# codenotary/immustore

Hardware: AMD Instinct MI355X
Metric: device-resident GiB/s hashed, htree build, 1M x 1KiB leaves (higher is better)
Workload: dtype u32; 1 GPU

## Files before the change

### immustore_amd/csrc/htree_kernels.hip

```cpp
#include <algorithm>
#include <cstring>

#include "mh_internal.hpp"
#include "sha256_cdna.hpp"
#include "digest_io.hpp"

typedef __attribute__((address_space(3))) void lds_void_t;
typedef __attribute__((address_space(1))) void glb_void_t;

namespace mh {

void LevelGeom::init(uint64_t n_) {
    n = n_;
    nlevels = 0;
    total = 0;
    for (int l = 0; l < kMaxLevels; l++) off[l] = width[l] = 0;
    if (n == 0) return;
    uint64_t w = n;
    for (;;) {
        off[nlevels] = total;
        width[nlevels] = w;
        total += w;
        nlevels++;
        if (w == 1) break;
        w = (w + 1) / 2;
    }
}

static LevelArgs level_args(const LevelGeom &g) {
    LevelArgs a;
    for (int l = 0; l < kMaxLevels; l++) {
        a.off[l] = g.off[l];
        a.width[l] = l < g.nlevels ? g.width[l] : 0;
    }
    return a;
}

void pad_block_kw(uint64_t len, KWTable *out) {
    static const uint32_t K[64] = {
        0x428a2f98u, 0x71374491u, 0xb5c0fbcfu, 0xe9b5dba5u, 0x3956c25bu, 0x59f111f1u, 0x923f82a4u,
        0xab1c5ed5u, 0xd807aa98u, 0x12835b01u, 0x243185beu, 0x550c7dc3u, 0x72be5d74u, 0x80deb1feu,
        0x9bdc06a7u, 0xc19bf174u, 0xe49b69c1u, 0xefbe4786u, 0x0fc19dc6u, 0x240ca1ccu, 0x2de92c6fu,
        0x4a7484aau, 0x5cb0a9dcu, 0x76f988dau, 0x983e5152u, 0xa831c66du, 0xb00327c8u, 0xbf597fc7u,
        0xc6e00bf3u, 0xd5a79147u, 0x06ca6351u, 0x14292967u, 0x27b70a85u, 0x2e1b2138u, 0x4d2c6dfcu,
        0x53380d13u, 0x650a7354u, 0x766a0abbu, 0x81c2c92eu, 0x92722c85u, 0xa2bfe8a1u, 0xa81a664bu,
        0xc24b8b70u, 0xc76c51a3u, 0xd192e819u, 0xd6990624u, 0xf40e3585u, 0x106aa070u, 0x19a4c116u,
        0x1e376c08u, 0x2748774cu, 0x34b0bcb5u, 0x391c0cb3u, 0x4ed8aa4au, 0x5b9cca4fu, 0x682e6ff3u,
        0x748f82eeu, 0x78a5636fu, 0x84c87814u, 0x8cc70208u, 0x90befffau, 0xa4506cebu, 0xbef9a3f7u,
        0xc67178f2u};
    auto ror = [](uint32_t x, int n) { return (x >> n) | (x << (32 - n)); };
    uint32_t w[64] = {0};
    uint64_t bits = len * 8;
    w[0] = 0x80000000u;
    w[14] = (uint32_t)(bits >> 32);
    w[15] = (uint32_t)bits;
    for (int t = 16; t < 64; t++) {
        uint32_t s0 = ror(w[t - 15], 7) ^ ror(w[t - 15], 18) ^ (w[t - 15] >> 3);
        uint32_t s1 = ror(w[t - 2], 17) ^ ror(w[t - 2], 19) ^ (w[t - 2] >> 10);
        w[t] = w[t - 16] + s0 + w[t - 7] + s1;
    }
    for (int t = 0; t < 64; t++) out->kw[t] = K[t] + w[t];
}

constexpr int kLaneLevels = 11;
struct LaneLevels {
    uint64_t off[kLaneLevels];
    uint64_t width[kLaneLevels];
};

static LaneLevels lane_levels(const LevelGeom &g) {
    LaneLevels a;
    for (int l = 0; l < kLaneLevels; l++) {
        a.off[l] = l < g.nlevels ? g.off[l] : 0;
        a.width[l] = l < g.nlevels ? g.width[l] : 0;
    }
    return a;
}

__device__ __forceinline__ void store_node(uint8_t *levels, const LaneLevels &la, int l, uint64_t q,
                                           const uint32_t w[8]) {
    if (q < la.width[l]) store_digest(levels + (la.off[l] + q) * 32, w);
}

template <int VER, int KW4>
__device__ __forceinline__ void digest_words(const uint32_t key[5], const uint32_t hv[8],
                                             uint32_t w[16]) {
    constexpr int P = VER == 1 ? 1 : 0;
    constexpr int L = (VER == 1 ? 4 : 0) + 4 * KW4 + 32;
#pragma unroll
    for (int j = 0; j < 16; j++) w[j] = 0;
    if (VER == 1) w[0] = 4 * KW4;
// ... 65 lines not shown
};

template <int LPL>
struct Log2 {
    static constexpr int v = LPL == 1 ? 0 : LPL == 2 ? 1 : 2;
};

constexpr int kFixedThreads = 256;
constexpr int kWaveLds = 8192;
constexpr uint32_t kFixedMaxValLen = 1u << 24;
constexpr uint32_t kFixedFastMaxValLen = 1u << 23;

#ifndef MH_WG_PROBE
#define MH_WG_PROBE(point)
#endif

__device__ __forceinline__ void dma_issue(const uint8_t *__restrict__ vals, uint32_t stride,
                                          uint64_t wave_slot0, int lpl, int i, uint64_t n,
                                          uint32_t byte_off, bool two, char *lds, int lane) {
    uint32_t ln = (uint32_t)lane;
    asm volatile("" : "+v"(ln));
    const uint64_t e0 = wave_slot0 * lpl;
    const uint32_t lim = (uint32_t)min<uint64_t>(n - 1 - e0, 0xffffffffull);
    const uint8_t *g0 = vals + e0 * stride + byte_off;
    if (two) {
        const uint32_t k2 = (ln & 7) ^ (ln >> 4);
#pragma unroll
        for (int j = 0; j < 8; j++) {
            const uint32_t rel = min((uint32_t)((j * 8 + (ln >> 3)) * lpl + i), lim);
            const uint32_t off = rel * stride + ((j & 1) ? (k2 ^ 4) : k2) * 16;
            __builtin_amdgcn_global_load_lds((glb_void_t *)(g0 + off),
                                             (lds_void_t *)(lds + j * 1024), 16, 0, 0);
        }
    } else {
        const uint32_t k1 = (ln & 3) ^ ((ln >> 4) & 3);
#pragma unroll
        for (int j = 0; j < 4; j++) {
            const uint32_t rel = min((uint32_t)((j * 16 + (ln >> 2)) * lpl + i), lim);
            const uint32_t off = rel * stride + k1 * 16;
            __builtin_amdgcn_global_load_lds((glb_void_t *)(g0 + off),
                                             (lds_void_t *)(lds + j * 1024), 16, 0, 0);
        }
    }
}

__device__ __forceinline__ void lds_block(const char *lds, int lane, bool two, int h,
                                          uint32_t w[16]) {
#pragma unroll
    for (int c = 0; c < 4; c++) {
        int addr;
        if (two) {
            const int k = 4 * h + c;
            addr = lane * 128 + ((k ^ ((lane >> 1) & 7)) << 4);
        } else {
            addr = lane * 64 + ((c ^ ((lane >> 2) & 3)) << 4);
        }
        const uint4 v = *reinterpret_cast<const uint4 *>(lds + addr);
        w[4 * c + 0] = bswap(v.x);
        w[4 * c + 1] = bswap(v.y);
        w[4 * c + 2] = bswap(v.z);
        w[4 * c + 3] = bswap(v.w);
    }
}

__device__ __forceinline__ void fast_lane_offsets(uint32_t stride, uint32_t lim, int lpl, int i,
                                                  int lane, uint32_t voff[8]) {
    const uint32_t ln = (uint32_t)lane;
    const uint32_t k2 = (ln & 7) ^ (ln >> 4);
#pragma unroll
    for (int j = 0; j < 8; j++) {
        const uint32_t rel = min((uint32_t)((j * 8 + (ln >> 3)) * lpl + i), lim);
        voff[j] = rel * stride + ((j & 1) ? (k2 ^ 4) : k2) * 16;
    }
}

__device__ __forceinline__ void dma_issue_fast(__amdgpu_buffer_rsrc_t rsrc, char *lds,
                                               const uint32_t voff[8], uint32_t byte_off) {
#pragma unroll
    for (int j = 0; j < 8; j++)
        __builtin_amdgcn_raw_ptr_buffer_load_lds(rsrc, (lds_void_t *)(lds + j * 1024), 16,
                                                 (int)voff[j], (int)byte_off, 0, 0);
}

__device__ __forceinline__ void lds_read4(const char *lds, uint32_t a, uint4 r[4]) {
#pragma unroll
    for (int c = 0; c < 4; c++) r[c] = *reinterpret_cast<const uint4 *>(lds + (a ^ (c << 4)));
}

__device__ __forceinline__ void swap_words(const uint4 r[4], uint32_t w[16]) {
#pragma unroll
    for (int c = 0; c < 4; c++) {
        w[4 * c + 0] = bswap(r[c].x);
        w[4 * c + 1] = bswap(r[c].y);
        w[4 * c + 2] = bswap(r[c].z);
        w[4 * c + 3] = bswap(r[c].w);
    }
}

enum : int { OP_VALUE = 0, OP_TAIL, OP_DIGEST, OP_LEAF, OP_NODE1, OP_NODE2 };

template <int LPL, bool FAST>
__global__ __launch_bounds__(kFixedThreads) void k_entries_fixed(
    const uint8_t *__restrict__ vals, uint32_t val_len, const uint8_t *__restrict__ keys,
    uint32_t key_len, int version, uint64_t n, uint8_t *__restrict__ hvals_out,
    uint8_t *__restrict__ levels, LaneLevels la, int wg_levels, KWTable kwt) {
    extern __shared__ __attribute__((aligned(16))) char smem[];
    const int lane = threadIdx.x & 63;
    int wave = threadIdx.x >> 6;
    if (FAST) wave = __builtin_amdgcn_readfirstlane(wave);
    uint32_t *kw_lds = reinterpret_cast<uint32_t *>(smem + (kFixedThreads / 64) * kWaveLds);
    if (FAST) {
        if (threadIdx.x < 64) kw_lds[threadIdx.x] = kwt.kw[threadIdx.x];
    } else if (threadIdx.x == 0) {
        uint32_t w[16];
#pragma unroll
        for (int j = 0; j < 16; j++) w[j] = 0;
        w[0] = 0x80000000u;
        const uint64_t bits = (uint64_t)val_len * 8;
        w[14] = (uint32_t)(bits >> 32);
        w[15] = (uint32_t)bits;
#pragma unroll
        for (int t = 0; t < 64; t++) {
            if (t >= 16)
                w[t & 15] = ssig1(w[(t - 2) & 15]) + w[(t - 7) & 15] + ssig0(w[(t - 15) & 15]) +
                            w[t & 15];
            kw_lds[t] = kK256[t] + w[t & 15];
        }
    }
    __syncthreads();
    MH_WG_PROBE(0);
    char *lds = smem + wave * kWaveLds;
    const uint64_t wave_slot0 = ((uint64_t)blockIdx.x * (kFixedThreads / 64) + wave) * 64;
    const uint64_t first = (wave_slot0 + lane) * LPL;
    const int c = first < n ? (int)min<uint64_t>(LPL, n - first) : 0;
    const bool wave_busy = wave_slot0 * LPL < n;

    const uint32_t nfull = val_len >> 6;
    const uint32_t rem = val_len & 63;
    const uint32_t nsteps2 = nfull >> 1;
    const uint32_t units = nsteps2 + (nfull & 1);
    const int kw4 = key_len >> 2;
    State s;
    s.init();
    uint32_t A[8], B[8], ny7 = 0;
    const bool fast_busy = FAST && wave_busy;
    const uint64_t e0 = fast_busy ? wave_slot0 * LPL : 0;
    const uint64_t ents = fast_busy ? n - e0 : 0;
    const uint32_t lim = ents - 1 < 0xffffffffull ? (uint32_t)(ents - 1) : 0xffffffffu;
    const uint64_t left = ents * val_len < 0xffffffffull ? ents * val_len : 0xffffffffull;
    const uint64_t base = (uint64_t)vals + e0 * val_len;
    const uint64_t base_s =
        ((uint64_t)(uint32_t)__builtin_amdgcn_readfirstlane((int)(uint32_t)(base >> 32)) << 32) |
        (uint32_t)__builtin_amdgcn_readfirstlane((int)(uint32_t)base);
    const __amdgpu_buffer_rsrc_t rsrc = __builtin_amdgcn_make_buffer_rsrc(
        (void *)base_s, 0, __builtin_amdgcn_readfirstlane((int)(uint32_t)left), 0x00020000);
    uint32_t voff[8];
    const uint32_t lds_a0 =
        (uint32_t)wave * kWaveLds + (uint32_t)lane * 128 + ((((uint32_t)lane >> 1) & 7) << 4);
    if (wave_busy) {
    if (FAST) {
        fast_lane_offsets(val_len, lim, LPL, 0, lane, voff);
        dma_issue_fast(rsrc, lds, voff, 0);
    } else {
    if (units) dma_issue(vals, val_len, wave_slot0, LPL, 0, n, 0, nsteps2 > 0, lds, lane);
    }

    int i = 0;
    uint32_t b = 0;
    int node = 0;
    int op = nfull ? OP_VALUE : (rem ? OP_TAIL : OP_DIGEST);
    if (!nfull && !rem && i < c) compress_kw(s, kw_lds);
    for (;;) {
        const uint64_t idx = first + i;
        bool on = i < c;
        if (op == OP_VALUE && FAST) {
#pragma unroll 1
            for (uint32_t bb = 0; bb < nfull; bb++) {
                uint4 r[4];
                uint32_t w[16];
                uint32_t a = lds_a0;
                asm volatile("" : "+v"(a));
                lds_read4(smem, a ^ ((bb & 1) << 6), r);
                if (bb & 1) {
                    asm volatile("s_waitcnt lgkmcnt(0)" ::: "memory");
                    const uint32_t u1 = (bb >> 1) + 1;
                    if (u1 < units) dma_issue_fast(rsrc, lds, voff, u1 * 128);
                }
                swap_words(r, w);
                compress(s, w);
                if (bb == 0 && i == 0) MH_WG_PROBE(3);
            }
            if (i + 1 < LPL) {
                fast_lane_offsets(val_len, lim, LPL, i + 1, lane, voff);
                dma_issue_fast(rsrc, lds, voff, 0);
            }
            if (on) compress_kw(s, kw_lds);
            op = OP_DIGEST;
            continue;
        }
        if (op == OP_VALUE) {
#pragma unroll 1
            for (; b < nfull; b++) {
                const uint32_t u = b >> 1;
                const bool two = u < nsteps2;
                const int h = two ? (int)(b & 1) : 0;
                uint32_t w[16];
                lds_block(lds, lane, two, h, w);
                if (!two || h == 1) {
                    asm volatile("s_waitcnt lgkmcnt(0)" ::: "memory");
                    if (u + 1 < units)
                        dma_issue(vals, val_len, wave_slot0, LPL, i, n, (u + 1) * 128,
                                  (u + 1) < nsteps2, lds, lane);
                    else if (i + 1 < LPL)
                        dma_issue(vals, val_len, wave_slot0, LPL, i + 1, n, 0, nsteps2 > 0, lds,
                                  lane);
                }
                if (on) compress(s, w);
                if (b == 0 && i == 0) MH_WG_PROBE(3);
            }
            b = 0;
            if (rem) {
                op = OP_TAIL;
            } else {
                if (on) compress_kw(s, kw_lds);
                op = OP_DIGEST;
            }
            continue;
        }
        uint32_t w[16];
        if (op == OP_TAIL) {
            const uint32_t rw = rem >> 2;
            const uint32_t *tp =
                reinterpret_cast<const uint32_t *>(vals + idx * val_len + (uint64_t)nfull * 64);
#pragma unroll
            for (int j = 0; j < 12; j++) w[j] = (on && j < (int)rw) ? bswap(tp[j]) : 0u;
#pragma unroll
            for (int j = 12; j < 16; j++) w[j] = 0;
#pragma unroll
            for (int j = 0; j < 13; j++)
                if (j == (int)rw) w[j] = 0x80000000u;
            const uint64_t bits = (uint64_t)val_len * 8;
            w[14] = (uint32_t)(bits >> 32);
            w[15] = (uint32_t)bits;
        } else if (op == OP_DIGEST) {
            if (on && hvals_out) store_digest(hvals_out + idx * 32, s.h);
            uint32_t key[5] = {0, 0, 0, 0, 0};
            const uint32_t *kp = reinterpret_cast<const uint32_t *>(keys + idx * key_len);
#pragma unroll
            for (int j = 0; j < 5; j++)
                if (on && j < kw4) key[j] = bswap(kp[j]);
            digest_block(version, kw4, key, s.h, w);
            s.init();
        } else if (op == OP_LEAF) {
            w[0] = s.h[0] >> 8;
#pragma unroll
            for (int j = 1; j < 8; j++) w[j] = __builtin_amdgcn_alignbit(s.h[j - 1], s.h[j], 8);
            w[8] = (s.h[7] << 24) | 0x00800000u;
#pragma unroll
            for (int j = 9; j < 15; j++) w[j] = 0;
            w[15] = 33u * 8u;
            s.init();
        } else if (op == OP_NODE1) {
            uint32_t l[8], r[8];
            if (LPL >= 2 && node == 0) {
#pragma unroll
                for (int j = 0; j < 8; j++) {
                    l[j] = i == 1 ? A[j] : B[j];
                    r[j] = s.h[j];
                }
                on = i < c;
            } else {
                copy8(l, A);
                copy8(r, B);
                on = c >= 3;
            }
            w[0] = 0x01000000u | (l[0] >> 8);
#pragma unroll
            for (int j = 1; j < 8; j++) w[j] = __builtin_amdgcn_alignbit(l[j - 1], l[j], 8);
            w[8] = __builtin_amdgcn_alignbit(l[7], r[0], 8);
#pragma unroll
            for (int j = 1; j < 8; j++) w[8 + j] = __builtin_amdgcn_alignbit(r[j - 1], r[j], 8);
            ny7 = r[7];
            s.init();
        } else {
            w[0] = (ny7 << 24) | 0x00800000u;
#pragma unroll
            for (int j = 1; j < 15; j++) w[j] = 0;
            w[15] = 65u * 8u;
            on = (node == 0) ? (i < c) : (c >= 3);
        }

        if (on) compress(s, w);

        bool entry_done = false;
        if (op == OP_TAIL) {
            op = OP_DIGEST;
        } else if (op == OP_DIGEST) {
            op = OP_LEAF;
        } else if (op == OP_LEAF) {
            if (i < c) store_digest(levels + idx * 32, s.h);
            if (LPL == 1) break;
            entry_done = true;
            if ((i & 1) == 0) {
#pragma unroll
                for (int j = 0; j < 8; j++) {
                    if (i == 0) A[j] = s.h[j];
                    else B[j] = s.h[j];
                }
            } else {
                node = 0;
                op = OP_NODE1;
                continue;
            }
        } else if (op == OP_NODE1) {
            op = OP_NODE2;
            continue;
        } else {
            const bool lane_on = (node == 0) ? (i < c) : (c >= 3);
            if (node == 0) {
#pragma unroll
                for (int j = 0; j < 8; j++) {
                    if (lane_on) {
                        if (i == 1) A[j] = s.h[j];
                        else B[j] = s.h[j];
                    }
                }
                if (c > 0) store_node(levels, la, 1, (first >> 1) + (i >> 1), i == 1 ? A : B);
                if (LPL == 4 && i == 3) {
                    node = 1;
                    op = OP_NODE1;
                    continue;
                }
            } else {
#pragma unroll
                for (int j = 0; j < 8; j++)
                    if (lane_on) A[j] = s.h[j];
            }
            if (LPL == 4 && i == 3 && c > 0) store_node(levels, la, 2, first >> 2, A);
            if (LPL == 2 || i == LPL - 1) break;
            entry_done = true;
        }
        if (entry_done) {
            if (++i >= LPL) break;
            s.init();
            op = nfull ? OP_VALUE : (rem ? OP_TAIL : OP_DIGEST);
            if (!nfull && !rem && i < c) compress_kw(s, kw_lds);
        }
    }
    }

    constexpr int L0 = LPL == 4 ? 2 : (LPL == 2 ? 1 : 0);
    MH_WG_PROBE(1);
    if (wg_levels == 0) return;
    const int t = threadIdx.x;
    uint32_t(*buf)[kFixedThreads][9] = reinterpret_cast<uint32_t(*)[kFixedThreads][9]>(smem);
    __syncthreads();
#pragma unroll
    for (int j = 0; j < 8; j++) buf[0][t][j] = LPL == 1 ? s.h[j] : A[j];
    int cur = 0;
#pragma unroll 1
    for (int st = 1; st <= wg_levels; st++) {
        __syncthreads();
        const int active = kFixedThreads >> st;
        const int l = L0 + st;
        if (t < active) {
            const uint64_t q = (uint64_t)blockIdx.x * active + t;
            if (q < la.width[l]) {
                uint32_t lft[8], rgt[8], out[8];
#pragma unroll
                for (int j = 0; j < 8; j++) lft[j] = buf[cur][2 * t][j];
                if (2 * q + 1 < la.width[l - 1]) {
#pragma unroll
                    for (int j = 0; j < 8; j++) rgt[j] = buf[cur][2 * t + 1][j];
                    node_hash(lft, rgt, out);
                } else {
                    copy8(out, lft);
                }
                store_digest(levels + (la.off[l] + q) * 32, out);
#pragma unroll
                for (int j = 0; j < 8; j++) buf[cur ^ 1][t][j] = out[j];
            }
        }
        cur ^= 1;
    }
    MH_WG_PROBE(2);
}

template <int LPL>
__global__ __launch_bounds__(256) void k_leaves_from_digests(const uint8_t *__restrict__ digests,
                                                             uint64_t n, uint8_t *__restrict__ levels,
                                                             LaneLevels la) {
    const uint64_t lane_id = (uint64_t)blockIdx.x * blockDim.x + threadIdx.x;
    const uint64_t first = lane_id * LPL;
    if (first >= n) return;
    const int c = (int)min<uint64_t>(LPL, n - first);
    LaneReducer<LPL> red;
#pragma unroll 1
    for (int i = 0; i < LPL; i++) {
        if (i < c) {
            uint32_t d[8], leaf[8];
            load_digest(digests + (first + i) * 32, d);
            leaf_hash(d, leaf);
            store_digest(levels + (first + i) * 32, leaf);
            red.push(i, leaf);
        }
    }
    red.finish(c, first, levels, la);
}

__global__ void k_copy_nodes(const uint8_t *__restrict__ src, uint64_t n, uint8_t *__restrict__ dst) {
    const uint64_t i = (uint64_t)blockIdx.x * blockDim.x + threadIdx.x;
    if (i < n * 2) reinterpret_cast<uint4 *>(dst)[i] = reinterpret_cast<const uint4 *>(src)[i];
}

template <int T>
__global__ __launch_bounds__(T) void k_reduce(uint8_t *__restrict__ levels, LevelArgs la, int l0,
                                              int nsteps, int top, uint8_t *__restrict__ root) {
    __shared__ uint32_t buf[2][T][9];
    const int t = threadIdx.x;
    const uint64_t blk = blockIdx.x;
    {
        const uint64_t q = blk * T + t;
        if (q < la.width[l0 + 1]) {
            uint32_t lft[8], rgt[8], out[8];
            load_digest(levels + (la.off[l0] + 2 * q) * 32, lft);
            if (2 * q + 1 < la.width[l0]) {
                load_digest(levels + (la.off[l0] + 2 * q + 1) * 32, rgt);
                node_hash_g(lft, rgt, out);
            } else {
                copy8(out, lft);
// ... 284 lines not shown
```

### immustore_amd/csrc/sha256_cdna.hpp

```cpp
#pragma once
#include <hip/hip_runtime.h>
#include <stdint.h>

namespace mh {

__device__ __constant__ static const uint32_t kK256[64] = {
    0x428a2f98u, 0x71374491u, 0xb5c0fbcfu, 0xe9b5dba5u, 0x3956c25bu, 0x59f111f1u, 0x923f82a4u,
    0xab1c5ed5u, 0xd807aa98u, 0x12835b01u, 0x243185beu, 0x550c7dc3u, 0x72be5d74u, 0x80deb1feu,
    0x9bdc06a7u, 0xc19bf174u, 0xe49b69c1u, 0xefbe4786u, 0x0fc19dc6u, 0x240ca1ccu, 0x2de92c6fu,
    0x4a7484aau, 0x5cb0a9dcu, 0x76f988dau, 0x983e5152u, 0xa831c66du, 0xb00327c8u, 0xbf597fc7u,
    0xc6e00bf3u, 0xd5a79147u, 0x06ca6351u, 0x14292967u, 0x27b70a85u, 0x2e1b2138u, 0x4d2c6dfcu,
    0x53380d13u, 0x650a7354u, 0x766a0abbu, 0x81c2c92eu, 0x92722c85u, 0xa2bfe8a1u, 0xa81a664bu,
    0xc24b8b70u, 0xc76c51a3u, 0xd192e819u, 0xd6990624u, 0xf40e3585u, 0x106aa070u, 0x19a4c116u,
    0x1e376c08u, 0x2748774cu, 0x34b0bcb5u, 0x391c0cb3u, 0x4ed8aa4au, 0x5b9cca4fu, 0x682e6ff3u,
    0x748f82eeu, 0x78a5636fu, 0x84c87814u, 0x8cc70208u, 0x90befffau, 0xa4506cebu, 0xbef9a3f7u,
    0xc67178f2u};

#define MH_K(i)                                                                                   \
    ((i) == 0 ? 0x428a2f98u : (i) == 1 ? 0x71374491u : (i) == 2 ? 0xb5c0fbcfu                   \
     : (i) == 3 ? 0xe9b5dba5u : (i) == 4 ? 0x3956c25bu : (i) == 5 ? 0x59f111f1u                  \
     : (i) == 6 ? 0x923f82a4u : (i) == 7 ? 0xab1c5ed5u : (i) == 8 ? 0xd807aa98u                  \
     : (i) == 9 ? 0x12835b01u : (i) == 10 ? 0x243185beu : (i) == 11 ? 0x550c7dc3u                \
     : (i) == 12 ? 0x72be5d74u : (i) == 13 ? 0x80deb1feu : (i) == 14 ? 0x9bdc06a7u               \
     : (i) == 15 ? 0xc19bf174u : (i) == 16 ? 0xe49b69c1u : (i) == 17 ? 0xefbe4786u               \
// ... 18 lines not shown
                                    0x510e527fu, 0x9b05688cu, 0x1f83d9abu, 0x5be0cd19u};

__device__ __forceinline__ uint32_t rotr(uint32_t x, uint32_t n) {
    return __builtin_amdgcn_alignbit(x, x, n);
}
__device__ __forceinline__ uint32_t xor3(uint32_t a, uint32_t b, uint32_t c) {
    return __builtin_amdgcn_bitop3_b32(a, b, c, 0x96);
}
__device__ __forceinline__ uint32_t bsig0(uint32_t a) { return xor3(rotr(a, 2), rotr(a, 13), rotr(a, 22)); }
__device__ __forceinline__ uint32_t bsig1(uint32_t e) { return xor3(rotr(e, 6), rotr(e, 11), rotr(e, 25)); }
__device__ __forceinline__ uint32_t ssig0(uint32_t x) { return xor3(rotr(x, 7), rotr(x, 18), x >> 3); }
__device__ __forceinline__ uint32_t ssig1(uint32_t x) { return xor3(rotr(x, 17), rotr(x, 19), x >> 10); }
__device__ __forceinline__ uint32_t ch(uint32_t e, uint32_t f, uint32_t g) {
    return __builtin_amdgcn_bitop3_b32(e, f, g, 0xCA);
}
__device__ __forceinline__ uint32_t maj(uint32_t a, uint32_t b, uint32_t c) {
    return __builtin_amdgcn_bitop3_b32(a, b, c, 0xE8);
}

__device__ __forceinline__ uint32_t bswap(uint32_t x) { return __builtin_bswap32(x); }

struct State {
    uint32_t h[8];
    __device__ __forceinline__ void init() {
#pragma unroll
        for (int i = 0; i < 8; i++) h[i] = kH0[i];
    }
};

#define MH_ROUND(a, b, c, d, e, f, g, h, kw)                                                      \
    do {                                                                                          \
        uint32_t t1_ = (h + (kw)) + (bsig1(e) + ch(e, f, g));                                     \
        d += t1_;                                                                                 \
        h = t1_ + (bsig0(a) + maj(a, b, c));                                                      \
    } while (0)

__device__ __forceinline__ void compress(State &s, const uint32_t win[16]) {
    uint32_t w[16];
#pragma unroll
    for (int i = 0; i < 16; i++) w[i] = win[i];
    uint32_t a = s.h[0], b = s.h[1], c = s.h[2], d = s.h[3], e = s.h[4], f = s.h[5], g = s.h[6],
             h = s.h[7];
#pragma unroll
    for (int r = 0; r < 64; r += 8) {
        if (r >= 16) {
#pragma unroll
            for (int j = 0; j < 8; j++) {
                const int t = r + j;
                w[t & 15] = ssig1(w[(t - 2) & 15]) + w[(t - 7) & 15] + ssig0(w[(t - 15) & 15]) +
                            w[t & 15];
            }
        }
        MH_ROUND(a, b, c, d, e, f, g, h, MH_K(r + 0) + w[(r + 0) & 15]);
        MH_ROUND(h, a, b, c, d, e, f, g, MH_K(r + 1) + w[(r + 1) & 15]);
        MH_ROUND(g, h, a, b, c, d, e, f, MH_K(r + 2) + w[(r + 2) & 15]);
        MH_ROUND(f, g, h, a, b, c, d, e, MH_K(r + 3) + w[(r + 3) & 15]);
        MH_ROUND(e, f, g, h, a, b, c, d, MH_K(r + 4) + w[(r + 4) & 15]);
        MH_ROUND(d, e, f, g, h, a, b, c, MH_K(r + 5) + w[(r + 5) & 15]);
        MH_ROUND(c, d, e, f, g, h, a, b, MH_K(r + 6) + w[(r + 6) & 15]);
        MH_ROUND(b, c, d, e, f, g, h, a, MH_K(r + 7) + w[(r + 7) & 15]);
    }
    s.h[0] += a; s.h[1] += b; s.h[2] += c; s.h[3] += d;
    s.h[4] += e; s.h[5] += f; s.h[6] += g; s.h[7] += h;
}

__device__ __forceinline__ void compress_kw(State &s, const uint32_t *__restrict__ kw) {
    uint32_t a = s.h[0], b = s.h[1], c = s.h[2], d = s.h[3], e = s.h[4], f = s.h[5], g = s.h[6],
             h = s.h[7];
#pragma unroll
    for (int r = 0; r < 64; r += 8) {
        MH_ROUND(a, b, c, d, e, f, g, h, kw[r + 0]);
        MH_ROUND(h, a, b, c, d, e, f, g, kw[r + 1]);
        MH_ROUND(g, h, a, b, c, d, e, f, kw[r + 2]);
        MH_ROUND(f, g, h, a, b, c, d, e, kw[r + 3]);
        MH_ROUND(e, f, g, h, a, b, c, d, kw[r + 4]);
        MH_ROUND(d, e, f, g, h, a, b, c, kw[r + 5]);
        MH_ROUND(c, d, e, f, g, h, a, b, kw[r + 6]);
        MH_ROUND(b, c, d, e, f, g, h, a, kw[r + 7]);
    }
    s.h[0] += a; s.h[1] += b; s.h[2] += c; s.h[3] += d;
    s.h[4] += e; s.h[5] += f; s.h[6] += g; s.h[7] += h;
}

__device__ __forceinline__ void leaf_hash(const uint32_t d[8], uint32_t out[8]) {
    uint32_t w[16];
    w[0] = d[0] >> 8;
#pragma unroll
    for (int j = 1; j < 8; j++) w[j] = __builtin_amdgcn_alignbit(d[j - 1], d[j], 8);
    w[8] = (d[7] << 24) | 0x00800000u;
#pragma unroll
    for (int j = 9; j < 15; j++) w[j] = 0;
    w[15] = 33u * 8u;
    State s;
    s.init();
    compress(s, w);
#pragma unroll
    for (int j = 0; j < 8; j++) out[j] = s.h[j];
}

__device__ __forceinline__ void node_hash(const uint32_t l[8], const uint32_t r[8], uint32_t out[8]) {
    uint32_t w[16];
    w[0] = 0x01000000u | (l[0] >> 8);
#pragma unroll
    for (int j = 1; j < 8; j++) w[j] = __builtin_amdgcn_alignbit(l[j - 1], l[j], 8);
    w[8] = __builtin_amdgcn_alignbit(l[7], r[0], 8);
#pragma unroll
    for (int j = 1; j < 8; j++) w[8 + j] = __builtin_amdgcn_alignbit(r[j - 1], r[j], 8);
    State s;
    s.init();
    compress(s, w);
    w[0] = (r[7] << 24) | 0x00800000u;
#pragma unroll
    for (int j = 1; j < 15; j++) w[j] = 0;
    w[15] = 65u * 8u;
    compress(s, w);
#pragma unroll
    for (int j = 0; j < 8; j++) out[j] = s.h[j];
}

constexpr int kNodeTabStride = 52;
constexpr int kNodeTabWords = 256 * kNodeTabStride;
constexpr int kNodeTabBytes = kNodeTabWords * 4;

struct alignas(16) NodeTab {
    uint32_t w[kNodeTabWords];
};

constexpr NodeTab make_node_tab() {
    constexpr uint32_t K[64] = {
        0x428a2f98u, 0x71374491u, 0xb5c0fbcfu, 0xe9b5dba5u, 0x3956c25bu, 0x59f111f1u, 0x923f82a4u,
        0xab1c5ed5u, 0xd807aa98u, 0x12835b01u, 0x243185beu, 0x550c7dc3u, 0x72be5d74u, 0x80deb1feu,
        0x9bdc06a7u, 0xc19bf174u, 0xe49b69c1u, 0xefbe4786u, 0x0fc19dc6u, 0x240ca1ccu, 0x2de92c6fu,
        0x4a7484aau, 0x5cb0a9dcu, 0x76f988dau, 0x983e5152u, 0xa831c66du, 0xb00327c8u, 0xbf597fc7u,
        0xc6e00bf3u, 0xd5a79147u, 0x06ca6351u, 0x14292967u, 0x27b70a85u, 0x2e1b2138u, 0x4d2c6dfcu,
        0x53380d13u, 0x650a7354u, 0x766a0abbu, 0x81c2c92eu, 0x92722c85u, 0xa2bfe8a1u, 0xa81a664bu,
        0xc24b8b70u, 0xc76c51a3u, 0xd192e819u, 0xd6990624u, 0xf40e3585u, 0x106aa070u, 0x19a4c116u,
        0x1e376c08u, 0x2748774cu, 0x34b0bcb5u, 0x391c0cb3u, 0x4ed8aa4au, 0x5b9cca4fu, 0x682e6ff3u,
        0x748f82eeu, 0x78a5636fu, 0x84c87814u, 0x8cc70208u, 0x90befffau, 0xa4506cebu, 0xbef9a3f7u,
        0xc67178f2u};
    NodeTab t{};
    for (uint32_t v = 0; v < 256; v++) {
        uint32_t w[64] = {};
        w[0] = (v << 24) | 0x00800000u;
        w[15] = 65u * 8u;
        for (int i = 16; i < 64; i++) {
            const uint32_t x = w[i - 15], y = w[i - 2];
            const uint32_t s0 = ((x >> 7) | (x << 25)) ^ ((x >> 18) | (x << 14)) ^ (x >> 3);
            const uint32_t s1 = ((y >> 17) | (y << 15)) ^ ((y >> 19) | (y << 13)) ^ (y >> 10);
            w[i] = s1 + w[i - 7] + s0 + w[i - 16];
            t.w[v * kNodeTabStride + (i - 16)] = w[i] + K[i];
        }
    }
    return t;
}

__device__ static const NodeTab g_node_tab = make_node_tab();

__device__ __forceinline__ void node_tab_init(uint32_t *tab) {
    const uint4 *src = (const uint4 *)g_node_tab.w;
    uint4 *dst = (uint4 *)tab;
    for (int i = threadIdx.x; i < kNodeTabWords / 4; i += blockDim.x) dst[i] = src[i];
    __syncthreads();
}

#define MH_ROUNDS8(k0, k1, k2, k3, k4, k5, k6, k7)                                                \
    do {                                                                                          \
        MH_ROUND(a, b, c, d, e, f, g, h, k0);                                                     \
        MH_ROUND(h, a, b, c, d, e, f, g, k1);                                                     \
        MH_ROUND(g, h, a, b, c, d, e, f, k2);                                                     \
        MH_ROUND(f, g, h, a, b, c, d, e, k3);                                                     \
        MH_ROUND(e, f, g, h, a, b, c, d, k4);                                                     \
        MH_ROUND(d, e, f, g, h, a, b, c, k5);                                                     \
        MH_ROUND(c, d, e, f, g, h, a, b, k6);                                                     \
        MH_ROUND(b, c, d, e, f, g, h, a, k7);                                                     \
    } while (0)

__device__ __forceinline__ void compress_node_tail(State &s, uint32_t r7,
                                                   const uint32_t *__restrict__ tab) {
    const uint4 *row = (const uint4 *)(tab + (r7 & 0xffu) * kNodeTabStride);
    uint32_t a = s.h[0], b = s.h[1], c = s.h[2], d = s.h[3], e = s.h[4], f = s.h[5], g = s.h[6],
             h = s.h[7];
    MH_ROUNDS8(MH_K(0) + ((r7 << 24) | 0x00800000u), MH_K(1), MH_K(2), MH_K(3), MH_K(4), MH_K(5),
               MH_K(6), MH_K(7));
    MH_ROUNDS8(MH_K(8), MH_K(9), MH_K(10), MH_K(11), MH_K(12), MH_K(13), MH_K(14),
               MH_K(15) + 65u * 8u);
#pragma unroll
    for (int q = 0; q < 6; q++) {
        const uint4 x = row[2 * q], y = row[2 * q + 1];
        MH_ROUNDS8(x.x, x.y, x.z, x.w, y.x, y.y, y.z, y.w);
    }
    s.h[0] += a; s.h[1] += b; s.h[2] += c; s.h[3] += d;
    s.h[4] += e; s.h[5] += f; s.h[6] += g; s.h[7] += h;
}

__device__ __forceinline__ void node_hash_tab(const uint32_t l[8], const uint32_t r[8],
                                              uint32_t out[8], const uint32_t *__restrict__ tab) {
    uint32_t w[16];
    w[0] = 0x01000000u | (l[0] >> 8);
// ... 67 lines not shown
```

Baseline: 1320 GiB/s.

## Split fast path into a dedicated single-compress-site state machine with explicit LDS addressing

The FAST specialization now has its own loop. Digest, leaf and node hashing are expressed as block builders (leaf_block, node_block1, node_block2) that feed one shared compress() call site, which shrinks code size and register pressure from the many inlined compress copies. LDS reads use explicit address-space-3 pointers computed from the smem base, and smem alignment is raised to 128. A conservative s_waitcnt vmcnt(0) is added before each LDS read, which may serialize the DMA prefetch and reduce load/compute overlap.

```diff
diff --git a/immustore_amd/csrc/htree_kernels.hip b/immustore_amd/csrc/htree_kernels.hip
--- a/immustore_amd/csrc/htree_kernels.hip
+++ b/immustore_amd/csrc/htree_kernels.hip
@@ -7,6 +7,8 @@
 
 typedef __attribute__((address_space(3))) void lds_void_t;
 typedef __attribute__((address_space(1))) void glb_void_t;
+typedef uint32_t u32x4_t __attribute__((ext_vector_type(4)));
+typedef __attribute__((address_space(3))) const u32x4_t lds_u32x4_t;
 
 namespace mh {
 
@@ -238,9 +240,12 @@
                                                  (int)voff[j], (int)byte_off, 0, 0);
 }
 
-__device__ __forceinline__ void lds_read4(const char *lds, uint32_t a, uint4 r[4]) {
-#pragma unroll
-    for (int c = 0; c < 4; c++) r[c] = *reinterpret_cast<const uint4 *>(lds + (a ^ (c << 4)));
+__device__ __forceinline__ void lds_read4(uint32_t a, uint4 r[4]) {
+#pragma unroll
+    for (int c = 0; c < 4; c++) {
+        const u32x4_t v = *(lds_u32x4_t *)(uintptr_t)(a ^ (c << 4));
+        r[c] = make_uint4(v.x, v.y, v.z, v.w);
+    }
 }
 
 __device__ __forceinline__ void swap_words(const uint4 r[4], uint32_t w[16]) {
@@ -260,7 +265,7 @@
     const uint8_t *__restrict__ vals, uint32_t val_len, const uint8_t *__restrict__ keys,
     uint32_t key_len, int version, uint64_t n, uint8_t *__restrict__ hvals_out,
     uint8_t *__restrict__ levels, LaneLevels la, int wg_levels, KWTable kwt) {
-    extern __shared__ __attribute__((aligned(16))) char smem[];
+    extern __shared__ __attribute__((aligned(128))) char smem[];
     const int lane = threadIdx.x & 63;
     int wave = threadIdx.x >> 6;
     if (FAST) wave = __builtin_amdgcn_readfirstlane(wave);
@@ -311,15 +316,118 @@
     const __amdgpu_buffer_rsrc_t rsrc = __builtin_amdgcn_make_buffer_rsrc(
         (void *)base_s, 0, __builtin_amdgcn_readfirstlane((int)(uint32_t)left), 0x00020000);
     uint32_t voff[8];
-    const uint32_t lds_a0 =
+    const uint32_t lds_a0 = (uint32_t)(uintptr_t)(lds_void_t *)smem +
         (uint32_t)wave * kWaveLds + (uint32_t)lane * 128 + ((((uint32_t)lane >> 1) & 7) << 4);
     if (wave_busy) {
     if (FAST) {
         fast_lane_offsets(val_len, lim, LPL, 0, lane, voff);
         dma_issue_fast(rsrc, lds, voff, 0);
+        int i = 0;
+        int node = 0;
+        int op = OP_DIGEST;
+        for (;;) {
+            const uint64_t idx = first + i;
+            const bool on = i < c;
+            uint32_t w[16];
+            if (op == OP_DIGEST) {
+                s.init();
+#pragma unroll 1
+                for (uint32_t bb = 0; bb < nfull; bb++) {
+                    uint4 r[4];
+                    uint32_t vw[16];
+                    asm volatile("s_waitcnt vmcnt(0)" ::: "memory");
+                    lds_read4(lds_a0 ^ ((bb & 1) << 6), r);
+                    if (bb & 1) {
+                        asm volatile("s_waitcnt lgkmcnt(0)" ::: "memory");
+                        const uint32_t u1 = (bb >> 1) + 1;
+                        if (u1 < units) dma_issue_fast(rsrc, lds, voff, u1 * 128);
+                    }
+                    swap_words(r, vw);
+                    compress(s, vw);
+                    if (bb == 0 && i == 0) MH_WG_PROBE(3);
+                }
+                if (i + 1 < LPL) {
+                    fast_lane_offsets(val_len, lim, LPL, i + 1, lane, voff);
+                    dma_issue_fast(rsrc, lds, voff, 0);
+                }
+                compress_kw(s, kw_lds);
+                if (on && hvals_out) store_digest(hvals_out + idx * 32, s.h);
+                uint32_t key[5] = {0, 0, 0, 0, 0};
+                const uint32_t *kp = reinterpret_cast<const uint32_t *>(keys + idx * key_len);
+#pragma unroll
+                for (int j = 0; j < 5; j++)
+                    if (on && j < kw4) key[j] = bswap(kp[j]);
+                digest_block(version, kw4, key, s.h, w);
+                s.init();
+            } else if (op == OP_LEAF) {
+                leaf_block(s.h, w);
+                s.init();
+            } else if (op == OP_NODE1) {
+                if (LPL == 4 && node == 1) {
+                    node_block1(A, B, w);
+                    ny7 = B[7];
+                } else {
+                    uint32_t l[8];
+#pragma unroll
+                    for (int j = 0; j < 8; j++) l[j] = (LPL == 2 || i == 1) ? A[j] : B[j];
+                    node_block1(l, s.h, w);
+                    ny7 = s.h[7];
+                }
+                s.init();
+            } else {
+                node_block2(ny7, w);
+            }
+
+            compress(s, w);
+
+            if (op == OP_DIGEST) {
+                op = OP_LEAF;
+            } else if (op == OP_LEAF) {
+                if (on) store_digest(levels + idx * 32, s.h);
+                if (LPL == 1) break;
+                if ((i & 1) == 0) {
+#pragma unroll
+                    for (int j = 0; j < 8; j++) {
+                        if (LPL == 2 || i == 0) A[j] = s.h[j];
+                        else B[j] = s.h[j];
+                    }
+                    i++;
+                    op = OP_DIGEST;
+                } else {
+                    node = 0;
+                    op = OP_NODE1;
+                }
+            } else if (op == OP_NODE1) {
+                op = OP_NODE2;
+            } else if (LPL == 4 && node == 1) {
+#pragma unroll
+                for (int j = 0; j < 8; j++)
+                    if (c >= 3) A[j] = s.h[j];
+                if (c > 0) store_node(levels, la, 2, first >> 2, A);
+                break;
+            } else {
+#pragma unroll
+                for (int j = 0; j < 8; j++) {
+                    if (on) {
+                        if (LPL == 2 || i == 1) A[j] = s.h[j];
+                        else B[j] = s.h[j];
+                    }
+                }
+                if (c > 0)
+                    store_node(levels, la, 1, (first >> 1) + (i >> 1),
+                               (LPL == 2 || i == 1) ? A : B);
+                if (LPL == 2) break;
+                if (i == 3) {
+                    node = 1;
+                    op = OP_NODE1;
+                } else {
+                    i++;
+                    op = OP_DIGEST;
+                }
+            }
+        }
     } else {
     if (units) dma_issue(vals, val_len, wave_slot0, LPL, 0, n, 0, nsteps2 > 0, lds, lane);
-    }
 
     int i = 0;
     uint32_t b = 0;
@@ -329,31 +437,6 @@
     for (;;) {
         const uint64_t idx = first + i;
         bool on = i < c;
-        if (op == OP_VALUE && FAST) {
-#pragma unroll 1
-            for (uint32_t bb = 0; bb < nfull; bb++) {
-                uint4 r[4];
-                uint32_t w[16];
-                uint32_t a = lds_a0;
-                asm volatile("" : "+v"(a));
-                lds_read4(smem, a ^ ((bb & 1) << 6), r);
-                if (bb & 1) {
-                    asm volatile("s_waitcnt lgkmcnt(0)" ::: "memory");
-                    const uint32_t u1 = (bb >> 1) + 1;
-                    if (u1 < units) dma_issue_fast(rsrc, lds, voff, u1 * 128);
-                }
-                swap_words(r, w);
-                compress(s, w);
-                if (bb == 0 && i == 0) MH_WG_PROBE(3);
-            }
-            if (i + 1 < LPL) {
-                fast_lane_offsets(val_len, lim, LPL, i + 1, lane, voff);
-                dma_issue_fast(rsrc, lds, voff, 0);
-            }
-            if (on) compress_kw(s, kw_lds);
-            op = OP_DIGEST;
-            continue;
-        }
         if (op == OP_VALUE) {
 #pragma unroll 1
             for (; b < nfull; b++) {
@@ -502,6 +585,7 @@
             op = nfull ? OP_VALUE : (rem ? OP_TAIL : OP_DIGEST);
             if (!nfull && !rem && i < c) compress_kw(s, kw_lds);
         }
+    }
     }
     }
 
diff --git a/immustore_amd/csrc/sha256_cdna.hpp b/immustore_amd/csrc/sha256_cdna.hpp
--- a/immustore_amd/csrc/sha256_cdna.hpp
+++ b/immustore_amd/csrc/sha256_cdna.hpp
@@ -124,8 +124,7 @@
     s.h[4] += e; s.h[5] += f; s.h[6] += g; s.h[7] += h;
 }
 
-__device__ __forceinline__ void leaf_hash(const uint32_t d[8], uint32_t out[8]) {
-    uint32_t w[16];
+__device__ __forceinline__ void leaf_block(const uint32_t d[8], uint32_t w[16]) {
     w[0] = d[0] >> 8;
 #pragma unroll
     for (int j = 1; j < 8; j++) w[j] = __builtin_amdgcn_alignbit(d[j - 1], d[j], 8);
@@ -133,6 +132,28 @@
 #pragma unroll
     for (int j = 9; j < 15; j++) w[j] = 0;
     w[15] = 33u * 8u;
+}
+
+__device__ __forceinline__ void node_block1(const uint32_t l[8], const uint32_t r[8],
+                                            uint32_t w[16]) {
+    w[0] = 0x01000000u | (l[0] >> 8);
+#pragma unroll
+    for (int j = 1; j < 8; j++) w[j] = __builtin_amdgcn_alignbit(l[j - 1], l[j], 8);
+    w[8] = __builtin_amdgcn_alignbit(l[7], r[0], 8);
+#pragma unroll
+    for (int j = 1; j < 8; j++) w[8 + j] = __builtin_amdgcn_alignbit(r[j - 1], r[j], 8);
+}
+
+__device__ __forceinline__ void node_block2(uint32_t r7, uint32_t w[16]) {
+    w[0] = (r7 << 24) | 0x00800000u;
+#pragma unroll
+    for (int j = 1; j < 15; j++) w[j] = 0;
+    w[15] = 65u * 8u;
+}
+
+__device__ __forceinline__ void leaf_hash(const uint32_t d[8], uint32_t out[8]) {
+    uint32_t w[16];
+    leaf_block(d, w);
     State s;
     s.init();
     compress(s, w);
@@ -142,19 +163,11 @@
 
 __device__ __forceinline__ void node_hash(const uint32_t l[8], const uint32_t r[8], uint32_t out[8]) {
     uint32_t w[16];
-    w[0] = 0x01000000u | (l[0] >> 8);
-#pragma unroll
-    for (int j = 1; j < 8; j++) w[j] = __builtin_amdgcn_alignbit(l[j - 1], l[j], 8);
-    w[8] = __builtin_amdgcn_alignbit(l[7], r[0], 8);
-#pragma unroll
-    for (int j = 1; j < 8; j++) w[8 + j] = __builtin_amdgcn_alignbit(r[j - 1], r[j], 8);
+    node_block1(l, r, w);
     State s;
     s.init();
     compress(s, w);
-    w[0] = (r[7] << 24) | 0x00800000u;
-#pragma unroll
-    for (int j = 1; j < 15; j++) w[j] = 0;
-    w[15] = 65u * 8u;
+    node_block2(r[7], w);
     compress(s, w);
 #pragma unroll
     for (int j = 0; j < 8; j++) out[j] = s.h[j];
```

Measured after the change: 1330 GiB/s (median of 6 runs). About the same (+0.8%).

## Split fast fixed-entry path into straight-line device function with noinline SHA block

Applied to the files above, without the earlier changes.

Moves the FAST path of the fixed-size entry kernel out of the op-driven state machine into a dedicated straight-line function. That function loops over leaves per lane, computes value, leaf and node digests directly, and then does the workgroup tree levels. Tail, key and node SHA compressions now go through a noinline sha_block call, so the compression body is instantiated once rather than inlined at every site. The aim is to cut code size, instruction cache pressure and register pressure, which may allow more waves per SIMD, at the cost of call overhead and register spills around the calls.

```diff
diff --git a/immustore_amd/csrc/htree_kernels.hip b/immustore_amd/csrc/htree_kernels.hip
--- a/immustore_amd/csrc/htree_kernels.hip
+++ b/immustore_amd/csrc/htree_kernels.hip
@@ -253,36 +253,15 @@
     }
 }
 
-enum : int { OP_VALUE = 0, OP_TAIL, OP_DIGEST, OP_LEAF, OP_NODE1, OP_NODE2 };
-
-template <int LPL, bool FAST>
-__global__ __launch_bounds__(kFixedThreads) void k_entries_fixed(
-    const uint8_t *__restrict__ vals, uint32_t val_len, const uint8_t *__restrict__ keys,
-    uint32_t key_len, int version, uint64_t n, uint8_t *__restrict__ hvals_out,
-    uint8_t *__restrict__ levels, LaneLevels la, int wg_levels, KWTable kwt) {
-    extern __shared__ __attribute__((aligned(16))) char smem[];
+template <int LPL>
+__device__ __forceinline__ void entries_fixed_fast(
+    const uint8_t *vals, uint32_t val_len, const uint8_t *keys, uint32_t key_len, int version,
+    uint64_t n, uint8_t *hvals_out, uint8_t *levels, const LaneLevels &la, int wg_levels,
+    const KWTable &kwt, char *smem) {
     const int lane = threadIdx.x & 63;
-    int wave = threadIdx.x >> 6;
-    if (FAST) wave = __builtin_amdgcn_readfirstlane(wave);
+    const int wave = __builtin_amdgcn_readfirstlane(threadIdx.x >> 6);
     uint32_t *kw_lds = reinterpret_cast<uint32_t *>(smem + (kFixedThreads / 64) * kWaveLds);
-    if (FAST) {
-        if (threadIdx.x < 64) kw_lds[threadIdx.x] = kwt.kw[threadIdx.x];
-    } else if (threadIdx.x == 0) {
-        uint32_t w[16];
-#pragma unroll
-        for (int j = 0; j < 16; j++) w[j] = 0;
-        w[0] = 0x80000000u;
-        const uint64_t bits = (uint64_t)val_len * 8;
-        w[14] = (uint32_t)(bits >> 32);
-        w[15] = (uint32_t)bits;
-#pragma unroll
-        for (int t = 0; t < 64; t++) {
-            if (t >= 16)
-                w[t & 15] = ssig1(w[(t - 2) & 15]) + w[(t - 7) & 15] + ssig0(w[(t - 15) & 15]) +
-                            w[t & 15];
-            kw_lds[t] = kK256[t] + w[t & 15];
-        }
-    }
+    if (threadIdx.x < 64) kw_lds[threadIdx.x] = kwt.kw[threadIdx.x];
     __syncthreads();
     MH_WG_PROBE(0);
     char *lds = smem + wave * kWaveLds;
@@ -292,16 +271,10 @@
     const bool wave_busy = wave_slot0 * LPL < n;
 
     const uint32_t nfull = val_len >> 6;
-    const uint32_t rem = val_len & 63;
-    const uint32_t nsteps2 = nfull >> 1;
-    const uint32_t units = nsteps2 + (nfull & 1);
+    const uint32_t units = nfull >> 1;
     const int kw4 = key_len >> 2;
-    State s;
-    s.init();
-    uint32_t A[8], B[8], ny7 = 0;
-    const bool fast_busy = FAST && wave_busy;
-    const uint64_t e0 = fast_busy ? wave_slot0 * LPL : 0;
-    const uint64_t ents = fast_busy ? n - e0 : 0;
+    const uint64_t e0 = wave_busy ? wave_slot0 * LPL : 0;
+    const uint64_t ents = wave_busy ? n - e0 : 0;
     const uint32_t lim = ents - 1 < 0xffffffffull ? (uint32_t)(ents - 1) : 0xffffffffu;
     const uint64_t left = ents * val_len < 0xffffffffull ? ents * val_len : 0xffffffffull;
     const uint64_t base = (uint64_t)vals + e0 * val_len;
@@ -310,26 +283,18 @@
         (uint32_t)__builtin_amdgcn_readfirstlane((int)(uint32_t)base);
     const __amdgpu_buffer_rsrc_t rsrc = __builtin_amdgcn_make_buffer_rsrc(
         (void *)base_s, 0, __builtin_amdgcn_readfirstlane((int)(uint32_t)left), 0x00020000);
-    uint32_t voff[8];
     const uint32_t lds_a0 =
         (uint32_t)wave * kWaveLds + (uint32_t)lane * 128 + ((((uint32_t)lane >> 1) & 7) << 4);
+    uint32_t node[8] = {0, 0, 0, 0, 0, 0, 0, 0};
     if (wave_busy) {
-    if (FAST) {
+        uint32_t voff[8];
+        uint32_t leaf[LPL][8];
         fast_lane_offsets(val_len, lim, LPL, 0, lane, voff);
         dma_issue_fast(rsrc, lds, voff, 0);
-    } else {
-    if (units) dma_issue(vals, val_len, wave_slot0, LPL, 0, n, 0, nsteps2 > 0, lds, lane);
-    }
-
-    int i = 0;
-    uint32_t b = 0;
-    int node = 0;
-    int op = nfull ? OP_VALUE : (rem ? OP_TAIL : OP_DIGEST);
-    if (!nfull && !rem && i < c) compress_kw(s, kw_lds);
-    for (;;) {
-        const uint64_t idx = first + i;
-        bool on = i < c;
-        if (op == OP_VALUE && FAST) {
+#pragma unroll 1
+        for (int i = 0; i < LPL; i++) {
+            State s;
+            s.init();
 #pragma unroll 1
             for (uint32_t bb = 0; bb < nfull; bb++) {
                 uint4 r[4];
@@ -350,10 +315,146 @@
                 fast_lane_offsets(val_len, lim, LPL, i + 1, lane, voff);
                 dma_issue_fast(rsrc, lds, voff, 0);
             }
-            if (on) compress_kw(s, kw_lds);
-            op = OP_DIGEST;
-            continue;
-        }
+            compress_kw(s, kw_lds);
+            const uint64_t idx = first + i;
+            const bool on = i < c;
+            if (on && hvals_out) store_digest(hvals_out + idx * 32, s.h);
+            uint32_t w[16];
+            uint32_t key[5] = {0, 0, 0, 0, 0};
+            const uint32_t *kp = reinterpret_cast<const uint32_t *>(keys + idx * key_len);
+#pragma unroll
+            for (int j = 0; j < 5; j++)
+                if (on && j < kw4) key[j] = bswap(kp[j]);
+            digest_block(version, kw4, key, s.h, w);
+            s.init();
+            sha_block(s, w);
+            w[0] = s.h[0] >> 8;
+#pragma unroll
+            for (int j = 1; j < 8; j++) w[j] = __builtin_amdgcn_alignbit(s.h[j - 1], s.h[j], 8);
+            w[8] = (s.h[7] << 24) | 0x00800000u;
+#pragma unroll
+            for (int j = 9; j < 15; j++) w[j] = 0;
+            w[15] = 33u * 8u;
+            s.init();
+            sha_block(s, w);
+            if (on) store_digest(levels + idx * 32, s.h);
+#pragma unroll
+            for (int k = 0; k + 1 < LPL; k++) copy8(leaf[k], leaf[k + 1]);
+            copy8(leaf[LPL - 1], s.h);
+        }
+        copy8(node, leaf[0]);
+        if constexpr (LPL >= 2) {
+            if (c >= 2) node_hash_call(leaf[0], leaf[1], node);
+            if (c > 0) store_node(levels, la, 1, first >> 1, node);
+        }
+        if constexpr (LPL == 4) {
+            if (c >= 3) {
+                uint32_t rgt[8];
+                copy8(rgt, leaf[2]);
+                if (c == 4) node_hash_call(leaf[2], leaf[LPL - 1], rgt);
+                store_node(levels, la, 1, (first >> 1) + 1, rgt);
+                node_hash_call(node, rgt, node);
+            }
+            if (c > 0) store_node(levels, la, 2, first >> 2, node);
+        }
+    }
+
+    constexpr int L0 = Log2<LPL>::v;
+    MH_WG_PROBE(1);
+    if (wg_levels == 0) return;
+    const int t = threadIdx.x;
+    uint32_t(*buf)[kFixedThreads][9] = reinterpret_cast<uint32_t(*)[kFixedThreads][9]>(smem);
+    __syncthreads();
+#pragma unroll
+    for (int j = 0; j < 8; j++) buf[0][t][j] = node[j];
+    int cur = 0;
+#pragma unroll 1
+    for (int st = 1; st <= wg_levels; st++) {
+        __syncthreads();
+        const int active = kFixedThreads >> st;
+        const int l = L0 + st;
+        if (t < active) {
+            const uint64_t q = (uint64_t)blockIdx.x * active + t;
+            if (q < la.width[l]) {
+                uint32_t lft[8], rgt[8], out[8];
+#pragma unroll
+                for (int j = 0; j < 8; j++) lft[j] = buf[cur][2 * t][j];
+                if (2 * q + 1 < la.width[l - 1]) {
+#pragma unroll
+                    for (int j = 0; j < 8; j++) rgt[j] = buf[cur][2 * t + 1][j];
+                    node_hash_call(lft, rgt, out);
+                } else {
+                    copy8(out, lft);
+                }
+                store_digest(levels + (la.off[l] + q) * 32, out);
+#pragma unroll
+                for (int j = 0; j < 8; j++) buf[cur ^ 1][t][j] = out[j];
+            }
+        }
+        cur ^= 1;
+    }
+    MH_WG_PROBE(2);
+}
+
+enum : int { OP_VALUE = 0, OP_TAIL, OP_DIGEST, OP_LEAF, OP_NODE1, OP_NODE2 };
+
+template <int LPL, bool FAST>
+__global__ __launch_bounds__(kFixedThreads) void k_entries_fixed(
+    const uint8_t *__restrict__ vals, uint32_t val_len, const uint8_t *__restrict__ keys,
+    uint32_t key_len, int version, uint64_t n, uint8_t *__restrict__ hvals_out,
+    uint8_t *__restrict__ levels, LaneLevels la, int wg_levels, KWTable kwt) {
+    extern __shared__ __attribute__((aligned(16))) char smem[];
+    if constexpr (FAST) {
+        entries_fixed_fast<LPL>(vals, val_len, keys, key_len, version, n, hvals_out, levels, la,
+                                wg_levels, kwt, smem);
+        return;
+    }
+    const int lane = threadIdx.x & 63;
+    const int wave = threadIdx.x >> 6;
+    uint32_t *kw_lds = reinterpret_cast<uint32_t *>(smem + (kFixedThreads / 64) * kWaveLds);
+    if (threadIdx.x == 0) {
+        uint32_t w[16];
+#pragma unroll
+        for (int j = 0; j < 16; j++) w[j] = 0;
+        w[0] = 0x80000000u;
+        const uint64_t bits = (uint64_t)val_len * 8;
+        w[14] = (uint32_t)(bits >> 32);
+        w[15] = (uint32_t)bits;
+#pragma unroll
+        for (int t = 0; t < 64; t++) {
+            if (t >= 16)
+                w[t & 15] = ssig1(w[(t - 2) & 15]) + w[(t - 7) & 15] + ssig0(w[(t - 15) & 15]) +
+                            w[t & 15];
+            kw_lds[t] = kK256[t] + w[t & 15];
+        }
+    }
+    __syncthreads();
+    MH_WG_PROBE(0);
+    char *lds = smem + wave * kWaveLds;
+    const uint64_t wave_slot0 = ((uint64_t)blockIdx.x * (kFixedThreads / 64) + wave) * 64;
+    const uint64_t first = (wave_slot0 + lane) * LPL;
+    const int c = first < n ? (int)min<uint64_t>(LPL, n - first) : 0;
+    const bool wave_busy = wave_slot0 * LPL < n;
+
+    const uint32_t nfull = val_len >> 6;
+    const uint32_t rem = val_len & 63;
+    const uint32_t nsteps2 = nfull >> 1;
+    const uint32_t units = nsteps2 + (nfull & 1);
+    const int kw4 = key_len >> 2;
+    State s;
+    s.init();
+    uint32_t A[8], B[8], ny7 = 0;
+    if (wave_busy) {
+    if (units) dma_issue(vals, val_len, wave_slot0, LPL, 0, n, 0, nsteps2 > 0, lds, lane);
+
+    int i = 0;
+    uint32_t b = 0;
+    int node = 0;
+    int op = nfull ? OP_VALUE : (rem ? OP_TAIL : OP_DIGEST);
+    if (!nfull && !rem && i < c) compress_kw(s, kw_lds);
+    for (;;) {
+        const uint64_t idx = first + i;
+        bool on = i < c;
         if (op == OP_VALUE) {
 #pragma unroll 1
             for (; b < nfull; b++) {
diff --git a/immustore_amd/csrc/sha256_cdna.hpp b/immustore_amd/csrc/sha256_cdna.hpp
--- a/immustore_amd/csrc/sha256_cdna.hpp
+++ b/immustore_amd/csrc/sha256_cdna.hpp
@@ -156,6 +156,56 @@
     for (int j = 1; j < 15; j++) w[j] = 0;
     w[15] = 65u * 8u;
     compress(s, w);
+#pragma unroll
+    for (int j = 0; j < 8; j++) out[j] = s.h[j];
+}
+
+typedef uint32_t u32x8 __attribute__((ext_vector_type(8)));
+typedef uint32_t u32x16 __attribute__((ext_vector_type(16)));
+
+static __device__ __attribute__((noinline)) u32x8 sha_block_regs(u32x8 h, u32x16 wv) {
+    State s;
+    uint32_t w[16];
+#pragma unroll
+    for (int j = 0; j < 8; j++) s.h[j] = h[j];
+#pragma unroll
+    for (int j = 0; j < 16; j++) w[j] = wv[j];
+    compress(s, w);
+#pragma unroll
+    for (int j = 0; j < 8; j++) h[j] = s.h[j];
+    return h;
+}
+
+__device__ __forceinline__ void sha_block(State &s, const uint32_t w[16]) {
+    u32x8 h;
+    u32x16 wv;
+#pragma unroll
+    for (int j = 0; j < 8; j++) h[j] = s.h[j];
+#pragma unroll
+    for (int j = 0; j < 16; j++) wv[j] = w[j];
+    h = sha_block_regs(h, wv);
+#pragma unroll
+    for (int j = 0; j < 8; j++) s.h[j] = h[j];
+}
+
+__device__ __forceinline__ void node_hash_call(const uint32_t l[8], const uint32_t r[8],
+                                               uint32_t out[8]) {
+    uint32_t w[16];
+    w[0] = 0x01000000u | (l[0] >> 8);
+#pragma unroll
+    for (int j = 1; j < 8; j++) w[j] = __builtin_amdgcn_alignbit(l[j - 1], l[j], 8);
+    w[8] = __builtin_amdgcn_alignbit(l[7], r[0], 8);
+#pragma unroll
+    for (int j = 1; j < 8; j++) w[8 + j] = __builtin_amdgcn_alignbit(r[j - 1], r[j], 8);
+    const uint32_t r7 = r[7];
+    State s;
+    s.init();
+    sha_block(s, w);
+    w[0] = (r7 << 24) | 0x00800000u;
+#pragma unroll
+    for (int j = 1; j < 15; j++) w[j] = 0;
+    w[15] = 65u * 8u;
+    sha_block(s, w);
 #pragma unroll
     for (int j = 0; j < 8; j++) out[j] = s.h[j];
 }
```

Result: faster. 1322 GiB/s before, 1348 GiB/s after, median of 6 (+1.9%).
